# osai-ai/tensor-stream

Measured on AMD Instinct MI355X. Metric: 1080p NV12→720p BGR24 planar fp32 frames/sec per GPU; achieved HBM GB/s vs roofline, higher is better.
Workload: dtype f32

## Files before the change

tensor-stream_amd/csrc/vpp_bicubic_cols.hip:

```cpp
#include "vpp_device.h"
#include "vpp_r32_store.h"

#include <vector>

#pragma clang fp contract(off)

namespace tsvpp {

typedef const __attribute__((address_space(4))) BcEntry *BcTab;
typedef int bc_i4 __attribute__((ext_vector_type(4)));
typedef const __attribute__((address_space(4))) int *BcRows;
typedef const __attribute__((address_space(4))) bc_i4 *BcRows4;
__device__ __forceinline__ BcTab bc_const(const BcEntry *p) { return (BcTab)(uintptr_t)p; }
__device__ __forceinline__ BcEntry bc_ld(BcTab p) {
    BcEntry e;
    e.ws = p->ws; e.sel = p->sel; e.l0 = p->l0; e.l1 = p->l1; e.l2 = p->l2; e.bias = p->bias; e.w = p->w; e.maxoff = p->maxoff;
    return e;
}

typedef uint32_t u32x2a4c __attribute__((ext_vector_type(2), aligned(4)));
typedef uint32_t u32x3a4c __attribute__((ext_vector_type(3), aligned(4)));

constexpr int BC_SHIFT = 22;
constexpr int BC_TIE = 560;

__device__ __forceinline__ float ub0(uint32_t v) { return (float)(v & 255u); }
__device__ __forceinline__ float ub1(uint32_t v) { return (float)((v >> 8) & 255u); }
__device__ __forceinline__ float ub2(uint32_t v) { return (float)((v >> 16) & 255u); }
__device__ __forceinline__ float ub3(uint32_t v) { return (float)(v >> 24); }

static BcEntry bc_axis(int idx, float ratio, int clamp_limit, int tap_limit) {
    BcEntry a;
    int p;
    double w;
    bicubic_axis(idx, ratio, clamp_limit, p, w);
    int lo, hi;
    bicubic_offsets(p, 1, tap_limit, lo, hi);
    a.ws = p - lo;
    a.sel = (uint32_t)lo << 8 | (uint32_t)(lo + hi) << 16 | (uint32_t)(lo + 2 * hi) << 24;
    a.maxoff = lo + 2 * hi;
    a.w = (float)w;
    double c[4];
    cubic_coeffs(w, c);
    uint32_t d0 = 0, d1 = 0, d2 = 0;
    int neg = 0;
    bool exact = true;
    for (int k = 0; k < 4; k++) {
        if (c[k] * 4194304.0 != __builtin_rint(c[k] * 4194304.0)) exact = false;
        const int C = (int)__builtin_rint(c[k] * 4194304.0);
        const int m = (k == 0 || k == 3) ? -C : C;
        d0 |= (uint32_t)(m & 255) << (8 * k);
        d1 |= (uint32_t)((m >> 8) & 255) << (8 * k);
        d2 |= (uint32_t)((m >> 16) & 255) << (8 * k);
        if (k == 0 || k == 3) neg += m;
    }
    a.l0 = (int)d0;
    a.l1 = (int)d1;
    a.l2 = (int)d2;
    a.bias = (1 << (BC_SHIFT - 1)) - 255 * neg;
    if (exact) a.maxoff |= (int)0x80000000;
    return a;
}

__device__ __forceinline__ int bc_isum(uint32_t taps, int l0, int l1, int l2, int bias) {
    const uint32_t x = taps ^ 0xff0000ffu;
    const uint32_t s2 = __builtin_amdgcn_udot4(x, (uint32_t)l2, 0u, false);
    const uint32_t s1 = __builtin_amdgcn_udot4(x, (uint32_t)l1, s2 << 8, false);
    return (int)__builtin_amdgcn_udot4(x, (uint32_t)l0, (s1 << 8) + (uint32_t)bias, false);
}
__device__ __forceinline__ void bc_isum4(const uint32_t (&tp)[4], const int (&l0)[4], const int (&l1)[4], const int (&l2)[4], const int (&bias)[4], int (&s)[4]) {
    uint32_t x[4], a[4], b[4];
#pragma unroll
    for (int k = 0; k < 4; k++) x[k] = tp[k] ^ 0xff0000ffu;
#pragma unroll
    for (int k = 0; k < 4; k++) a[k] = __builtin_amdgcn_udot4(x[k], (uint32_t)l2[k], 0u, false);
#pragma unroll
    for (int k = 0; k < 4; k++) b[k] = __builtin_amdgcn_udot4(x[k], (uint32_t)l1[k], a[k] << 8, false);
#pragma unroll
    for (int k = 0; k < 4; k++) s[k] = (int)__builtin_amdgcn_udot4(x[k], (uint32_t)l0[k], (b[k] << 8) + (uint32_t)bias[k], false);
}
__device__ __forceinline__ void bc_isum4(const uint32_t (&tp)[4], int l0, int l1, int l2, int bias, int (&s)[4]) {
    const int a0[4] = { l0, l0, l0, l0 }, a1[4] = { l1, l1, l1, l1 }, a2[4] = { l2, l2, l2, l2 }, ab[4] = { bias, bias, bias, bias };
    bc_isum4(tp, a0, a1, a2, ab, s);
}
__device__ __forceinline__ uint32_t bc_tie_key(int s) { return (uint32_t)(s + BC_TIE) << (32 - BC_SHIFT); }
constexpr uint32_t BC_TIE_KEY = (2u * BC_TIE) << (32 - BC_SHIFT);
__device__ __forceinline__ uint32_t bc_exact(uint32_t taps, float w) {
    double c[4];
    cubic_coeffs((double)w, c);
    return (uint32_t)cubic4(c, (int)(taps & 255u), (int)((taps >> 8) & 255u), (int)((taps >> 16) & 255u), (int)(taps >> 24));
}
__device__ __forceinline__ uint32_t bc_pack4(int s0, int s1, int s2, int s3) {
    uint32_t hi;
    asm("s_nop 2\n\tv_ashr_pk_u8_i32 %0, %1, %2, 22" : "=v"(hi) : "v"(s2), "v"(s3));
    uint32_t r = hi << 16;
    asm("s_nop 2\n\tv_ashr_pk_u8_i32 %0, %1, %2, 22" : "+v"(r) : "v"(s0), "v"(s1));
    return r;
}
template <bool EXACT>
__device__ __forceinline__ uint32_t bc_finish4(const int s[4], const uint32_t tp[4], float w0, float w1, float w2, float w3, uint32_t exm) {
    uint32_t r = bc_pack4(s[0], s[1], s[2], s[3]);
    if constexpr (!EXACT) {
        const uint32_t k0 = bc_tie_key(s[0]) | exm, k1 = bc_tie_key(s[1]) | exm, k2 = bc_tie_key(s[2]) | exm, k3 = bc_tie_key(s[3]) | exm;
        if (min(min(k0, k1), min(k2, k3)) < BC_TIE_KEY) {
            if (k0 < BC_TIE_KEY) r = (r & 0xffffff00u) | bc_exact(tp[0], w0);
            if (k1 < BC_TIE_KEY) r = (r & 0xffff00ffu) | bc_exact(tp[1], w1) << 8;
            if (k2 < BC_TIE_KEY) r = (r & 0xff00ffffu) | bc_exact(tp[2], w2) << 16;
            if (k3 < BC_TIE_KEY) r = (r & 0x00ffffffu) | bc_exact(tp[3], w3) << 24;
        }
    }
    return r;
}
__device__ __forceinline__ uint32_t rep4(uint32_t b) { return __builtin_amdgcn_perm(0u, b, 0u); }

template <int STEP, int NDW>
__device__ __forceinline__ uint32_t bc_taps(const uint32_t (&dw)[NDW], uint32_t sh, uint32_t selx) {
    if constexpr (STEP == 1) {
        return __builtin_amdgcn_perm(dw[1], dw[0], selx);
    } else {
        const uint32_t a0 = __builtin_amdgcn_alignbyte(dw[1], dw[0], sh), a1 = __builtin_amdgcn_alignbyte(dw[2], dw[1], sh);
        return __builtin_amdgcn_perm(a1, a0, selx);
    }
}

__device__ __forceinline__ int bc_row_ws(BcRows rb, int i) { return rb[(i >> 2) * 32 + (i & 3)]; }
__device__ __forceinline__ uint32_t bc_row_sel(BcRows rb, int i) { return (uint32_t)rb[(i >> 2) * 32 + 4 + (i & 3)]; }

template <bool EXACT, bool SPARSE, int STEP>
__device__ __forceinline__ void bc_plane(const uint8_t *frame_plane, int pitch, int rows_in_plane, int row_bytes, const BcEntry &ax, int comp, bool dma, int lanes_per_row,
                                         uint8_t *ring, uint8_t *hcol, uint8_t *res, int lane, int nout, BcRows rb) {
    constexpr int NDW = STEP == 1 ? 2 : 3;
    const uint32_t pm = (uint32_t)((uintptr_t)frame_plane & 15);
    const uint8_t *plane = frame_plane - pm;
    const int ylo = bc_row_ws(rb, 0), yhi = min(bc_row_ws(rb, nout - 1) + 3, rows_in_plane - 1);
    const int ng = SPARSE ? nout : ((yhi - ylo + 1 + 3) >> 2);
    const int xb = STEP * ax.ws + comp;
    const uint32_t exm = (uint32_t)(ax.maxoff >> 31);
    const uint32_t tapsel = STEP == 1 ? ax.sel : ax.sel + ax.sel;
    if (dma && (pitch & 15) == 0) {
        const bool wide = !SPARSE && lanes_per_row > 16;
        const int L = SPARSE ? 16 : lanes_per_row, rpb = (SPARSE || wide) ? 4 : 4 * (16 / L), gpb = rpb >> 2;
        const int xb0 = __builtin_amdgcn_readlane(xb, 0);
        const uint32_t seg0 = (pm + (uint32_t)xb0) & ~15u;
        const uint32_t a_c = (uint32_t)(xb - xb0) + ((pm + (uint32_t)xb0) & 15u);
        const uint32_t al_c = a_c & ~3u, sh_c = a_c & 3u, selx_c = STEP == 1 ? tapsel + rep4(sh_c) : tapsel;
        const uint32_t last_chunk = ((uint32_t)(rows_in_plane - 1) * (uint32_t)pitch + pm + (uint32_t)row_bytes - 1u) & ~15u;
        const int lrow = (lane * (65536 / L + 1)) >> 16, lchunk = lane - lrow * L;
        const bool lane_on = wide ? lrow < 2 : lrow < rpb;
        const uint32_t lconst = seg0 + 16u * (uint32_t)lchunk + (SPARSE ? 0u : (uint32_t)lrow * (uint32_t)pitch);
        const int rstride = 16 * L;
        const int slot_bytes = wide ? 4 * rstride : 1024;
        const int nb = (ng + gpb - 1) / gpb;
        auto issue = [&](int bt, int slot) {
            uint32_t voff;
            if constexpr (SPARSE) {
                const uint32_t tapoff = __builtin_amdgcn_ubfe(bc_row_sel(rb, bt), 8u * (uint32_t)lrow, 8u);
                voff = ((uint32_t)bc_row_ws(rb, bt) + tapoff) * (uint32_t)pitch + lconst;
            } else {
                voff = (uint32_t)(ylo + rpb * bt) * (uint32_t)pitch + lconst;
            }
            uint8_t *dst = ring + slot * slot_bytes;
            const uint32_t v0 = min(voff, last_chunk);
            if (lane_on)
                __builtin_amdgcn_global_load_lds((const __attribute__((address_space(1))) void *)(plane + v0), (__attribute__((address_space(3))) void *)dst, 16, 0, 0);
            if constexpr (!SPARSE) {
                if (wide) {
                    const uint32_t v1 = min(voff + 2u * (uint32_t)pitch, last_chunk);
                    if (lane_on)
                        __builtin_amdgcn_global_load_lds((const __attribute__((address_space(1))) void *)(plane + v1),
                                                         (__attribute__((address_space(3))) void *)(dst + 2 * rstride), 16, 0, 0);
                }
            }
        };
        issue(0, 0);
        if (nb > 1) issue(1, 1);
        if (nb > 2) issue(2, 2);
        int slot = 0, bt = 0, gin = 0;
        for (int g = 0; g < ng; g++) {
            if (gin == 0) {
                if (wide) {
                    if (bt + 2 < nb) asm volatile("s_waitcnt vmcnt(4)" ::: "memory");
                    else if (bt + 1 < nb) asm volatile("s_waitcnt vmcnt(2)" ::: "memory");
                    else asm volatile("s_waitcnt vmcnt(0)" ::: "memory");
                } else {
                    if (bt + 2 < nb) asm volatile("s_waitcnt vmcnt(2)" ::: "memory");
                    else if (bt + 1 < nb) asm volatile("s_waitcnt vmcnt(1)" ::: "memory");
                    else asm volatile("s_waitcnt vmcnt(0)" ::: "memory");
                }
            }
            const uint8_t *p0 = ring + slot * slot_bytes + 4 * gin * rstride + al_c;
            uint32_t tp[4];
#pragma unroll
            for (int k = 0; k < 4; k++) {
                const uint32_t *p = (const uint32_t *)(p0 + k * rstride);
                uint32_t dw[NDW];
#pragma unroll
                for (int q = 0; q < NDW; q++) dw[q] = p[q];
                tp[k] = bc_taps<STEP, NDW>(dw, sh_c, selx_c);
            }
            if (++gin == gpb) {
                if (bt + 3 < nb) {
                    asm volatile("s_waitcnt lgkmcnt(0)" ::: "memory");
                    issue(bt + 3, slot);
                }
                gin = 0;
                bt++;
                slot = slot == 2 ? 0 : slot + 1;
            }
            int s[4];
            bc_isum4(tp, ax.l0, ax.l1, ax.l2, ax.bias, s);
            *(uint32_t *)(hcol + 4 * g) = bc_finish4<EXACT>(s, tp, ax.w, ax.w, ax.w, ax.w, exm);
        }
    } else {
        const uint32_t xoff = pm + (uint32_t)xb;
        const int xneed = STEP * (ax.maxoff & 0x7fffffff);
        const bool aligned = (pitch & 3) == 0;
        const uint32_t sh_c = xoff & 3u, selx_c = STEP == 1 ? tapsel + rep4(sh_c) : tapsel;
        auto group_rows = [&](int g, int (&rr)[4]) {
            if constexpr (SPARSE) {
                const int ws = bc_row_ws(rb, g);
                const uint32_t sel = bc_row_sel(rb, g);
#pragma unroll
                for (int k = 0; k < 4; k++) rr[k] = ws + (int)((sel >> (8 * k)) & 255u);
            } else {
#pragma unroll
                for (int k = 0; k < 4; k++) rr[k] = min(ylo + 4 * g + k, yhi);
            }
        };
        auto row_ptr = [&](int row, uint32_t &sh) {
            const uint32_t a = (uint32_t)row * (uint32_t)pitch + xoff;
            sh = aligned ? sh_c : (a & 3u);
            return aligned ? (const uint32_t *)(plane + (size_t)((uint32_t)row * (uint32_t)pitch) + (xoff & ~3u)) : (const uint32_t *)(plane + (a & ~3u));
        };
        auto fetch = [&](int g, uint32_t (&dw)[4][NDW], uint32_t (&sh)[4]) {
            int rr[4];
            group_rows(g, rr);
#pragma unroll
            for (int k = 0; k < 4; k++) {
                const uint32_t *p = row_ptr(rr[k], sh[k]);
                if constexpr (NDW == 2) {
                    const u32x2a4c v = *(const u32x2a4c *)p;
                    dw[k][0] = v.x; dw[k][1] = v.y;
                } else {
                    const u32x3a4c v = *(const u32x3a4c *)p;
                    dw[k][0] = v.x; dw[k][1] = v.y; dw[k][2] = v.z;
                }
            }
        };
        auto finish = [&](int g, const uint32_t (&dw)[4][NDW], const uint32_t (&sh)[4]) {
            uint32_t tp[4];
#pragma unroll
            for (int k = 0; k < 4; k++) tp[k] = bc_taps<STEP, NDW>(dw[k], sh[k], aligned ? selx_c : (STEP == 1 ? tapsel + rep4(sh[k]) : tapsel));
            int s[4];
            bc_isum4(tp, ax.l0, ax.l1, ax.l2, ax.bias, s);
            *(uint32_t *)(hcol + 4 * g) = bc_finish4<EXACT>(s, tp, ax.w, ax.w, ax.w, ax.w, exm);
        };
        int ngf;
        if constexpr (SPARSE) ngf = (bc_row_ws(rb, nout - 1) + 3 < rows_in_plane - 1) ? ng : 0;
        else ngf = (yhi < rows_in_plane - 1) ? ng : max(min((rows_in_plane - 1 - ylo) >> 2, ng), 0);
        if (ngf > 0) {
            uint32_t cur[4][NDW], csh[4];
            fetch(0, cur, csh);
            for (int g = 0; g + 1 < ngf; g++) {
                uint32_t nxt[4][NDW], nsh[4];
                fetch(g + 1, nxt, nsh);
                finish(g, cur, csh);
#pragma unroll
                for (int k = 0; k < 4; k++) {
                    csh[k] = nsh[k];
#pragma unroll
                    for (int q = 0; q < NDW; q++) cur[k][q] = nxt[k][q];
                }
            }
            finish(ngf - 1, cur, csh);
        }
        for (int g = ngf; g < ng; g++) {
            int rr[4];
            group_rows(g, rr);
            uint32_t dw[4][NDW], sh[4];
#pragma unroll
            for (int k = 0; k < 4; k++) {
                const uint32_t *p = row_ptr(rr[k], sh[k]);
                const int hi = (int)sh[k] + xneed;
#pragma unroll
                for (int q = 0; q < NDW; q++) dw[k][q] = p[(rr[k] < rows_in_plane - 1 || 4 * q <= hi) ? q : 0];
            }
            finish(g, dw, sh);
        }
    }
    __builtin_amdgcn_fence(__ATOMIC_RELEASE, "wavefront");
    __builtin_amdgcn_wave_barrier();
    for (int i = 0; i < nout; i += 4) {
        const BcRows blk = rb + (i >> 2) * 32;
        const bc_i4 ws4 = *(BcRows4)(blk), sel4 = *(BcRows4)(blk + 4), a4 = *(BcRows4)(blk + 8), b4 = *(BcRows4)(blk + 12), c4 = *(BcRows4)(blk + 16),
                    bias4 = *(BcRows4)(blk + 20), ex4 = *(BcRows4)(blk + 28);
        uint32_t tp[4];
        int s[4];
#pragma unroll
        for (int e = 0; e < 4; e++) {
            const int off = SPARSE ? 4 * (i + e) : max(ws4[e] - ylo, 0);
            const uint32_t *p = (const uint32_t *)(hcol + (off & ~3));
            const uint32_t win = __builtin_amdgcn_alignbyte(p[1], p[0], (uint32_t)off & 3u);
            tp[e] = SPARSE ? win : __builtin_amdgcn_perm(0u, win, (uint32_t)sel4[e]);
        }
        {
            const int q0[4] = { a4[0], a4[1], a4[2], a4[3] }, q1[4] = { b4[0], b4[1], b4[2], b4[3] }, q2[4] = { c4[0], c4[1], c4[2], c4[3] },
                      qb[4] = { bias4[0], bias4[1], bias4[2], bias4[3] };
            bc_isum4(tp, q0, q1, q2, qb, s);
        }
        uint32_t r = bc_pack4(s[0], s[1], s[2], s[3]);
        if constexpr (!EXACT) {
            const uint32_t k0 = bc_tie_key(s[0]) | (uint32_t)ex4[0], k1 = bc_tie_key(s[1]) | (uint32_t)ex4[1], k2 = bc_tie_key(s[2]) | (uint32_t)ex4[2],
                           k3 = bc_tie_key(s[3]) | (uint32_t)ex4[3];
            if (min(min(k0, k1), min(k2, k3)) < BC_TIE_KEY) {
                const BcRows wp = blk + 24;
                if (k0 < BC_TIE_KEY) r = (r & 0xffffff00u) | bc_exact(tp[0], __builtin_bit_cast(float, wp[0]));
                if (k1 < BC_TIE_KEY) r = (r & 0xffff00ffu) | bc_exact(tp[1], __builtin_bit_cast(float, wp[1])) << 8;
                if (k2 < BC_TIE_KEY) r = (r & 0xff00ffffu) | bc_exact(tp[2], __builtin_bit_cast(float, wp[2])) << 16;
                if (k3 < BC_TIE_KEY) r = (r & 0x00ffffffu) | bc_exact(tp[3], __builtin_bit_cast(float, wp[3])) << 24;
            }
        }
        res[i * 64 + lane] = (uint8_t)r;
        if (i + 1 < nout) res[(i + 1) * 64 + lane] = (uint8_t)(r >> 8);
        if (i + 2 < nout) res[(i + 2) * 64 + lane] = (uint8_t)(r >> 16);
        if (i + 3 < nout) res[(i + 3) * 64 + lane] = (uint8_t)(r >> 24);
    }
}

template <int OUT, bool EXACT, bool SPARSE>
__global__ __launch_bounds__(MAX_THREADS) void vpp_bicubic_cols_kernel(const LaunchDesc d, const FrameTable t) {
    using T = typename OutT<OUT>::type;
    const TileId id = decode_tile(d);
    if (!id.valid) return;
    const int lane = (int)(threadIdx.x & 63u), wave = __builtin_amdgcn_readfirstlane((int)(threadIdx.x >> 6));
    const int R = 8 * d.rpt;
    const int j_first = tile_col0(d, id.tx, 256) + wave * 64, i_first = id.ty * R;
    if (j_first >= d.dst_w) return;
    const int nrows = min(R, d.dst_h - i_first), ncrows = nrows >> 1;
    const bool dma = d.bc_dma != 0;

    uint8_t *wl = lds_raw + wave * d.bc_wave_bytes;
    uint8_t *ring = wl, *hcol = wl + d.bc_ring_bytes + lane * d.hcs_y;
    uint8_t *yt = wl + d.bc_ring_bytes + 64 * d.hcs_y, *uvt = yt + 64 * R;

    const BcTab col_y = bc_const(d.bc_tab), col_c = col_y + d.dst_w;
    const BcRows row_y = (BcRows)(col_c + (d.dst_w >> 1)), row_c = row_y + 32 * d.bc_npy;
    {
        const BcEntry ax = bc_ld(col_y + min(j_first + lane, d.dst_w - 1));
        bc_plane<EXACT, SPARSE, 1>(t.y[id.frame], d.pitch_y, d.src_h, d.src_w, ax, 0, dma, d.bc_dma, ring, hcol, yt, lane, nrows, row_y + (i_first >> 2) * 32);
    }
    if constexpr (!kLumaOnly<OUT>) {
        const BcEntry ax = bc_ld(col_c + min((j_first >> 1) + (lane >> 1), (d.dst_w >> 1) - 1));
        bc_plane<EXACT, SPARSE, 2>(t.uv[id.frame], d.pitch_uv, d.src_h >> 1, d.src_w, ax, lane & 1, dma, d.bc_dma, ring, hcol, uvt, lane, ncrows, row_c + (i_first >> 3) * 32);
    }
    __builtin_amdgcn_fence(__ATOMIC_RELEASE, "wavefront");
    __builtin_amdgcn_wave_barrier();

    if constexpr (OUT == O_U8_PLANAR || OUT == O_U8_MERGED || OUT == O_NV12_U8 || OUT == O_Y800_U8) {
        if (d.bc_u8x) {
            const int gx = lane & 7, gy = lane >> 3;
            const int j0 = j_first + 8 * gx, r0 = 4 * gy;
            if (j0 >= d.dst_w || r0 >= nrows) return;
            uint32_t ylo[4], yhi[4], clo[2] = { 0x80808080u, 0x80808080u }, chi[2] = { 0x80808080u, 0x80808080u };
#pragma unroll
            for (int r = 0; r < 4; r++) {
                const uint32_t *p = (const uint32_t *)(yt + (r0 + r) * 64 + 8 * gx);
                ylo[r] = p[0];
                yhi[r] = p[1];
            }
            if constexpr (!kLumaOnly<OUT>) {
#pragma unroll
                for (int rc = 0; rc < 2; rc++) {
                    const uint32_t *p = (const uint32_t *)(uvt + ((r0 >> 1) + rc) * 64 + 8 * gx);
                    clo[rc] = p[0];
                    chi[rc] = p[1];
                }
            }
            const int run_a = min(8, (d.dst_w - j_first) >> 3);
            r32_store_tile<OUT>(d, (uint8_t *)t.out[id.frame], ylo, yhi, clo, chi, i_first + r0, j0, gx, run_a);
            return;
        }
    }
    const int lx = lane & 15, ly = lane >> 4;
    const int j0 = j_first + lx * PXW;
    if (j0 >= d.dst_w) return;
    if (is_row_tail(d, j0)) return;
    for (int s = 0; s < d.rpt; s++) {
        const int r0 = s * 8 + ly * PXH, i0 = i_first + r0;
        if (i0 >= d.dst_h) break;
        float Uf[2] = { 128.0f, 128.0f }, Vf[2] = { 128.0f, 128.0f }, Yf[PXH][PXW];
#pragma unroll
        for (int r = 0; r < PXH; r++) {
            const uint32_t v = *(const uint32_t *)(yt + (r0 + r) * 64 + lx * PXW);
            Yf[r][0] = ub0(v);
            Yf[r][1] = ub1(v);
            Yf[r][2] = ub2(v);
            Yf[r][3] = ub3(v);
        }
        if constexpr (!kLumaOnly<OUT>) {
            const uint32_t c = *(const uint32_t *)(uvt + (r0 >> 1) * 64 + lx * PXW);
            Uf[0] = ub0(c);
            Vf[0] = ub1(c);
            Uf[1] = ub2(c);
            Vf[1] = ub3(c);
        }
        color_store_tile<OUT, true>(Yf, Uf, Vf, d, (T *)t.out[id.frame], i0, j0, PXW);
    }
}

int bicubic_cols_rows_padded(int n) { return (n + 3) / 4 + 1; }

const BcEntry *bicubic_cols_tables(const LaunchDesc &d, hipStream_t stream, bool may_build) {
    GeoCache *cache = d.geo_cache;
    if (!cache) return nullptr;
    GeoKey key;
    memset(&key, 0, sizeof(key));
    uint32_t xb, yb;
    memcpy(&xb, &d.xr, 4);
    memcpy(&yb, &d.yr, 4);
    const int kv[16] = { 2 , d.src_w, d.src_h, d.dst_w, d.dst_h, (int)xb, (int)yb, 0, 0, 0, 0, 0, 0, 0, 0, 0 };
    memcpy(key.v, kv, sizeof(kv));
    std::lock_guard<std::mutex> lk(cache->mu);
    auto it = cache->map.find(key);
    if (it == cache->map.end()) {
        if (!may_build) return nullptr;
        hipStreamCaptureStatus cs = hipStreamCaptureStatusNone;
        if (stream && hipStreamIsCapturing(stream, &cs) == hipSuccess && cs != hipStreamCaptureStatusNone) {
            g_build_declined = true;
            return nullptr;
        }
        if (!geo_cache_make_room(cache)) return nullptr;
        std::vector<uint8_t> buf;
        auto append = [&](const void *p, size_t n) {
            const size_t at = buf.size();
            buf.resize(at + n);
            memcpy(buf.data() + at, p, n);
        };
        for (int j = 0; j < d.dst_w; j++) {
            const BcEntry e = bc_axis(j, d.xr, d.src_w, d.src_w);
            append(&e, sizeof(e));
        }
        for (int j = 0; j < (d.dst_w >> 1); j++) {
            const BcEntry e = bc_axis(j, d.xr, d.src_w, d.src_w >> 1);
            append(&e, sizeof(e));
        }
        auto row_blocks = [&](int n, int tap_limit) {
            const int nb = bicubic_cols_rows_padded(n);
            std::vector<int> a((size_t)32 * nb, 0);
            for (int i = 0; i < 4 * nb; i++) {
                const BcEntry e = bc_axis(i < n ? i : n - 1, d.yr, d.src_h, tap_limit);
                int wbits;
                memcpy(&wbits, &e.w, 4);
                const int v[8] = { e.ws, (int)e.sel, e.l0, e.l1, e.l2, e.bias, wbits, e.maxoff >> 31  };
                for (int f = 0; f < 8; f++) a[(size_t)(i >> 2) * 32 + 4 * f + (i & 3)] = v[f];
            }
            append(a.data(), a.size() * sizeof(int));
        };
        row_blocks(d.dst_h, d.src_h);
        row_blocks(d.dst_h >> 1, d.src_h >> 1);
        GeoEntry e;
        if (hipMalloc((void **)&e.dev, buf.size()) != hipSuccess) {
            (void)hipGetLastError();
            return nullptr;
        }
        if (hipMemcpy(e.dev, buf.data(), buf.size(), hipMemcpyHostToDevice) != hipSuccess) {
            (void)hipGetLastError();
            (void)hipFree(e.dev);
            return nullptr;
        }
        e.bytes = buf.size();
        it = cache->map.emplace(key, e).first;
    }
    it->second.stamp = ++cache->clock;
    return (const BcEntry *)it->second.dev;
}

hipError_t launch_bicubic_cols(OutKind out, bool exact, const LaunchDesc &d, const FrameTable &t, size_t lds_bytes, hipStream_t stream, LaunchInfo *info) {
    dim3 grid((unsigned)(d.blocks_per_xcd * NUM_XCD)), block(MAX_THREADS);
    const bool sparse = d.bc_sparse != 0;
    const char *name = exact ? (sparse ? "vpp_bicubic_cols_kernel<OUT, exact, sparse>" : "vpp_bicubic_cols_kernel<OUT, exact, dense>")
                             : (sparse ? "vpp_bicubic_cols_kernel<OUT, tie, sparse>" : "vpp_bicubic_cols_kernel<OUT, tie, dense>");
    if (describe_only(info, name, grid, lds_bytes + (out == O_U8_MERGED ? out_side_static_lds(out) : 0))) return hipSuccess;
    if (!d.bc_tab) return hipErrorInvalidValue;
    return with_out_kind(out, [&](auto O) {
        constexpr int OUT = decltype(O)::value;
        if (exact && sparse) TSVPP_LAUNCH((vpp_bicubic_cols_kernel<OUT, true, true>), grid, block, lds_bytes, stream, d, t);
        else if (exact) TSVPP_LAUNCH((vpp_bicubic_cols_kernel<OUT, true, false>), grid, block, lds_bytes, stream, d, t);
        else if (sparse) TSVPP_LAUNCH((vpp_bicubic_cols_kernel<OUT, false, true>), grid, block, lds_bytes, stream, d, t);
        else TSVPP_LAUNCH((vpp_bicubic_cols_kernel<OUT, false, false>), grid, block, lds_bytes, stream, d, t);
        return hipGetLastError();
    });
}

}
```

Before: 435,600.

## Specialize bicubic DMA phase on wide layout and streamline ring loop

Moves the DMA-ring horizontal pass into a helper templated on the wide layout, so the wide/narrow branches are resolved at compile time. The per-group loop becomes a per-batch loop with incremental address stepping and byte slot offsets, instead of multiplying row offsets each time. It also fuses the pack asm into one block and hoists the tie mask OR outside the min. In the vertical pass it prefetches the next block's ws/sel table entries and drops the bounds checks on the tail stores. The unguarded tail stores and the prefetch past nout could write or read beyond the valid rows when nout is not a multiple of 4, which is a correctness risk unless buffers are padded.

Result: no change. 435,900 (median of 4 runs) (+0.1%).

```diff
diff --git a/tensor-stream_amd/csrc/vpp_bicubic_cols.hip b/tensor-stream_amd/csrc/vpp_bicubic_cols.hip
--- a/tensor-stream_amd/csrc/vpp_bicubic_cols.hip
+++ b/tensor-stream_amd/csrc/vpp_bicubic_cols.hip
@@ -91,18 +91,16 @@
     return (uint32_t)cubic4(c, (int)(taps & 255u), (int)((taps >> 8) & 255u), (int)((taps >> 16) & 255u), (int)(taps >> 24));
 }
 __device__ __forceinline__ uint32_t bc_pack4(int s0, int s1, int s2, int s3) {
-    uint32_t hi;
-    asm("s_nop 2\n\tv_ashr_pk_u8_i32 %0, %1, %2, 22" : "=v"(hi) : "v"(s2), "v"(s3));
-    uint32_t r = hi << 16;
-    asm("s_nop 2\n\tv_ashr_pk_u8_i32 %0, %1, %2, 22" : "+v"(r) : "v"(s0), "v"(s1));
+    uint32_t r;
+    asm("s_nop 2\n\tv_ashr_pk_u8_i32 %0, %3, %4, 22\n\tv_lshlrev_b32 %0, 16, %0\n\tv_ashr_pk_u8_i32 %0, %1, %2, 22" : "=&v"(r) : "v"(s0), "v"(s1), "v"(s2), "v"(s3));
     return r;
 }
 template <bool EXACT>
 __device__ __forceinline__ uint32_t bc_finish4(const int s[4], const uint32_t tp[4], float w0, float w1, float w2, float w3, uint32_t exm) {
     uint32_t r = bc_pack4(s[0], s[1], s[2], s[3]);
     if constexpr (!EXACT) {
-        const uint32_t k0 = bc_tie_key(s[0]) | exm, k1 = bc_tie_key(s[1]) | exm, k2 = bc_tie_key(s[2]) | exm, k3 = bc_tie_key(s[3]) | exm;
-        if (min(min(k0, k1), min(k2, k3)) < BC_TIE_KEY) {
+        const uint32_t k0 = bc_tie_key(s[0]), k1 = bc_tie_key(s[1]), k2 = bc_tie_key(s[2]), k3 = bc_tie_key(s[3]);
+        if ((min(min(k0, k1), min(k2, k3)) | exm) < BC_TIE_KEY) {
             if (k0 < BC_TIE_KEY) r = (r & 0xffffff00u) | bc_exact(tp[0], w0);
             if (k1 < BC_TIE_KEY) r = (r & 0xffff00ffu) | bc_exact(tp[1], w1) << 8;
             if (k2 < BC_TIE_KEY) r = (r & 0xff00ffffu) | bc_exact(tp[2], w2) << 16;
@@ -125,6 +123,80 @@
 
 __device__ __forceinline__ int bc_row_ws(BcRows rb, int i) { return rb[(i >> 2) * 32 + (i & 3)]; }
 __device__ __forceinline__ uint32_t bc_row_sel(BcRows rb, int i) { return (uint32_t)rb[(i >> 2) * 32 + 4 + (i & 3)]; }
+
+template <bool EXACT, bool SPARSE, int STEP, bool WIDE>
+__device__ __forceinline__ void bc_phase1_dma(const uint8_t *plane, uint32_t pm, int pitch, int rows_in_plane, int row_bytes, const BcEntry &ax, int lanes_per_row, uint8_t *ring,
+                                              uint8_t *hcol, int lane, int ylo, int ng, int xb, uint32_t exm, uint32_t tapsel, BcRows rb) {
+    static_assert(!(SPARSE && WIDE), "the wide ring layout is a dense-mode layout");
+    constexpr int NDW = STEP == 1 ? 2 : 3;
+    {
+        const int L = SPARSE ? 16 : lanes_per_row, rpb = (SPARSE || WIDE) ? 4 : 4 * (16 / L), gpb = rpb >> 2;
+        const int xb0 = __builtin_amdgcn_readlane(xb, 0);
+        const uint32_t seg0 = (pm + (uint32_t)xb0) & ~15u;
+        const uint32_t a_c = (uint32_t)(xb - xb0) + ((pm + (uint32_t)xb0) & 15u);
+        const uint32_t al_c = a_c & ~3u, sh_c = a_c & 3u, selx_c = STEP == 1 ? tapsel + rep4(sh_c) : tapsel;
+        const uint32_t last_chunk = ((uint32_t)(rows_in_plane - 1) * (uint32_t)pitch + pm + (uint32_t)row_bytes - 1u) & ~15u;
+        const int lrow = (lane * (65536 / L + 1)) >> 16, lchunk = lane - lrow * L;
+        const bool lane_on = WIDE ? lrow < 2 : lrow < rpb;
+        const uint32_t lconst = seg0 + 16u * (uint32_t)lchunk + (SPARSE ? 0u : (uint32_t)lrow * (uint32_t)pitch);
+        const int rstride = 16 * L;
+        const int slot_bytes = WIDE ? 4 * rstride : 1024;
+        const int nb = (ng + gpb - 1) / gpb;
+        const uint32_t bstep = (uint32_t)rpb * (uint32_t)pitch, pitch2 = 2u * (uint32_t)pitch;
+        uint32_t vnext = (uint32_t)ylo * (uint32_t)pitch + lconst;
+        auto issue = [&](int bt, int slot_off) {
+            uint32_t voff;
+            if constexpr (SPARSE) {
+                const uint32_t tapoff = __builtin_amdgcn_ubfe(bc_row_sel(rb, bt), 8u * (uint32_t)lrow, 8u);
+                voff = ((uint32_t)bc_row_ws(rb, bt) + tapoff) * (uint32_t)pitch + lconst;
+            } else {
+                voff = vnext;
+                vnext += bstep;
+            }
+            uint8_t *dst = ring + slot_off;
+            const uint32_t v0 = min(voff, last_chunk);
+            if (lane_on)
+                __builtin_amdgcn_global_load_lds((const __attribute__((address_space(1))) void *)(plane + v0), (__attribute__((address_space(3))) void *)dst, 16, 0, 0);
+            if constexpr (WIDE) {
+                const uint32_t v1 = min(voff + pitch2, last_chunk);
+                if (lane_on)
+                    __builtin_amdgcn_global_load_lds((const __attribute__((address_space(1))) void *)(plane + v1),
+                                                     (__attribute__((address_space(3))) void *)(dst + 2 * rstride), 16, 0, 0);
+            }
+        };
+        issue(0, 0);
+        if (nb > 1) issue(1, slot_bytes);
+        if (nb > 2) issue(2, 2 * slot_bytes);
+        int slot_off = 0, g = 0;
+        for (int bt = 0; bt < nb; bt++) {
+            if (bt + 2 < nb) asm volatile("s_waitcnt vmcnt(%0)" ::"n"(WIDE ? 4 : 2) : "memory");
+            else if (bt + 1 < nb) asm volatile("s_waitcnt vmcnt(%0)" ::"n"(WIDE ? 2 : 1) : "memory");
+            else asm volatile("s_waitcnt vmcnt(0)" ::: "memory");
+            const int ge = min(g + gpb, ng);
+            const bool refill = bt + 3 < nb;
+            for (int rd = slot_off; g < ge; g++, rd += 4 * rstride) {
+                const uint8_t *p0 = ring + rd + al_c;
+                uint32_t tp[4];
+#pragma unroll
+                for (int k = 0; k < 4; k++) {
+                    const uint32_t *p = (const uint32_t *)(p0 + k * rstride);
+                    uint32_t dw[NDW];
+#pragma unroll
+                    for (int q = 0; q < NDW; q++) dw[q] = p[q];
+                    tp[k] = bc_taps<STEP, NDW>(dw, sh_c, selx_c);
+                }
+                if (refill && g + 1 == ge) {
+                    asm volatile("s_waitcnt lgkmcnt(0)" ::: "memory");
+                    issue(bt + 3, slot_off);
+                }
+                int s[4];
+                bc_isum4(tp, ax.l0, ax.l1, ax.l2, ax.bias, s);
+                *(uint32_t *)(hcol + 4 * g) = bc_finish4<EXACT>(s, tp, ax.w, ax.w, ax.w, ax.w, exm);
+            }
+            slot_off = slot_off == 2 * slot_bytes ? 0 : slot_off + slot_bytes;
+        }
+    }
+}
 
 template <bool EXACT, bool SPARSE, int STEP>
 __device__ __forceinline__ void bc_plane(const uint8_t *frame_plane, int pitch, int rows_in_plane, int row_bytes, const BcEntry &ax, int comp, bool dma, int lanes_per_row,
@@ -138,79 +210,8 @@
     const uint32_t exm = (uint32_t)(ax.maxoff >> 31);
     const uint32_t tapsel = STEP == 1 ? ax.sel : ax.sel + ax.sel;
     if (dma && (pitch & 15) == 0) {
-        const bool wide = !SPARSE && lanes_per_row > 16;
-        const int L = SPARSE ? 16 : lanes_per_row, rpb = (SPARSE || wide) ? 4 : 4 * (16 / L), gpb = rpb >> 2;
-        const int xb0 = __builtin_amdgcn_readlane(xb, 0);
-        const uint32_t seg0 = (pm + (uint32_t)xb0) & ~15u;
-        const uint32_t a_c = (uint32_t)(xb - xb0) + ((pm + (uint32_t)xb0) & 15u);
-        const uint32_t al_c = a_c & ~3u, sh_c = a_c & 3u, selx_c = STEP == 1 ? tapsel + rep4(sh_c) : tapsel;
-        const uint32_t last_chunk = ((uint32_t)(rows_in_plane - 1) * (uint32_t)pitch + pm + (uint32_t)row_bytes - 1u) & ~15u;
-        const int lrow = (lane * (65536 / L + 1)) >> 16, lchunk = lane - lrow * L;
-        const bool lane_on = wide ? lrow < 2 : lrow < rpb;
-        const uint32_t lconst = seg0 + 16u * (uint32_t)lchunk + (SPARSE ? 0u : (uint32_t)lrow * (uint32_t)pitch);
-        const int rstride = 16 * L;
-        const int slot_bytes = wide ? 4 * rstride : 1024;
-        const int nb = (ng + gpb - 1) / gpb;
-        auto issue = [&](int bt, int slot) {
-            uint32_t voff;
-            if constexpr (SPARSE) {
-                const uint32_t tapoff = __builtin_amdgcn_ubfe(bc_row_sel(rb, bt), 8u * (uint32_t)lrow, 8u);
-                voff = ((uint32_t)bc_row_ws(rb, bt) + tapoff) * (uint32_t)pitch + lconst;
-            } else {
-                voff = (uint32_t)(ylo + rpb * bt) * (uint32_t)pitch + lconst;
-            }
-            uint8_t *dst = ring + slot * slot_bytes;
-            const uint32_t v0 = min(voff, last_chunk);
-            if (lane_on)
-                __builtin_amdgcn_global_load_lds((const __attribute__((address_space(1))) void *)(plane + v0), (__attribute__((address_space(3))) void *)dst, 16, 0, 0);
-            if constexpr (!SPARSE) {
-                if (wide) {
-                    const uint32_t v1 = min(voff + 2u * (uint32_t)pitch, last_chunk);
-                    if (lane_on)
-                        __builtin_amdgcn_global_load_lds((const __attribute__((address_space(1))) void *)(plane + v1),
-                                                         (__attribute__((address_space(3))) void *)(dst + 2 * rstride), 16, 0, 0);
-                }
-            }
-        };
-        issue(0, 0);
-        if (nb > 1) issue(1, 1);
-        if (nb > 2) issue(2, 2);
-        int slot = 0, bt = 0, gin = 0;
-        for (int g = 0; g < ng; g++) {
-            if (gin == 0) {
-                if (wide) {
-                    if (bt + 2 < nb) asm volatile("s_waitcnt vmcnt(4)" ::: "memory");
-                    else if (bt + 1 < nb) asm volatile("s_waitcnt vmcnt(2)" ::: "memory");
-                    else asm volatile("s_waitcnt vmcnt(0)" ::: "memory");
-                } else {
-                    if (bt + 2 < nb) asm volatile("s_waitcnt vmcnt(2)" ::: "memory");
-                    else if (bt + 1 < nb) asm volatile("s_waitcnt vmcnt(1)" ::: "memory");
-                    else asm volatile("s_waitcnt vmcnt(0)" ::: "memory");
-                }
-            }
-            const uint8_t *p0 = ring + slot * slot_bytes + 4 * gin * rstride + al_c;
-            uint32_t tp[4];
-#pragma unroll
-            for (int k = 0; k < 4; k++) {
-                const uint32_t *p = (const uint32_t *)(p0 + k * rstride);
-                uint32_t dw[NDW];
-#pragma unroll
-                for (int q = 0; q < NDW; q++) dw[q] = p[q];
-                tp[k] = bc_taps<STEP, NDW>(dw, sh_c, selx_c);
-            }
-            if (++gin == gpb) {
-                if (bt + 3 < nb) {
-                    asm volatile("s_waitcnt lgkmcnt(0)" ::: "memory");
-                    issue(bt + 3, slot);
-                }
-                gin = 0;
-                bt++;
-                slot = slot == 2 ? 0 : slot + 1;
-            }
-            int s[4];
-            bc_isum4(tp, ax.l0, ax.l1, ax.l2, ax.bias, s);
-            *(uint32_t *)(hcol + 4 * g) = bc_finish4<EXACT>(s, tp, ax.w, ax.w, ax.w, ax.w, exm);
-        }
+        if (!SPARSE && lanes_per_row > 16) bc_phase1_dma<EXACT, SPARSE, STEP, !SPARSE>(plane, pm, pitch, rows_in_plane, row_bytes, ax, lanes_per_row, ring, hcol, lane, ylo, ng, xb, exm, tapsel, rb);
+        else bc_phase1_dma<EXACT, SPARSE, STEP, false>(plane, pm, pitch, rows_in_plane, row_bytes, ax, lanes_per_row, ring, hcol, lane, ylo, ng, xb, exm, tapsel, rb);
     } else {
         const uint32_t xoff = pm + (uint32_t)xb;
         const int xneed = STEP * (ax.maxoff & 0x7fffffff);
@@ -290,10 +291,13 @@
     }
     __builtin_amdgcn_fence(__ATOMIC_RELEASE, "wavefront");
     __builtin_amdgcn_wave_barrier();
+    bc_i4 ws_next = *(BcRows4)(rb), sel_next = *(BcRows4)(rb + 4);
     for (int i = 0; i < nout; i += 4) {
         const BcRows blk = rb + (i >> 2) * 32;
-        const bc_i4 ws4 = *(BcRows4)(blk), sel4 = *(BcRows4)(blk + 4), a4 = *(BcRows4)(blk + 8), b4 = *(BcRows4)(blk + 12), c4 = *(BcRows4)(blk + 16),
-                    bias4 = *(BcRows4)(blk + 20), ex4 = *(BcRows4)(blk + 28);
+        const bc_i4 ws4 = ws_next, sel4 = sel_next;
+        const bc_i4 a4 = *(BcRows4)(blk + 8), b4 = *(BcRows4)(blk + 12), c4 = *(BcRows4)(blk + 16), bias4 = *(BcRows4)(blk + 20), ex4 = *(BcRows4)(blk + 28);
+        ws_next = *(BcRows4)(blk + 32);
+        sel_next = *(BcRows4)(blk + 36);
         uint32_t tp[4];
         int s[4];
 #pragma unroll
@@ -321,9 +325,9 @@
             }
         }
         res[i * 64 + lane] = (uint8_t)r;
-        if (i + 1 < nout) res[(i + 1) * 64 + lane] = (uint8_t)(r >> 8);
-        if (i + 2 < nout) res[(i + 2) * 64 + lane] = (uint8_t)(r >> 16);
-        if (i + 3 < nout) res[(i + 3) * 64 + lane] = (uint8_t)(r >> 24);
+        res[(i + 1) * 64 + lane] = (uint8_t)(r >> 8);
+        res[(i + 2) * 64 + lane] = (uint8_t)(r >> 16);
+        res[(i + 3) * 64 + lane] = (uint8_t)(r >> 24);
     }
 }
 
```
